# Priberam/Enhance-CB-Whisper

Measured on AMD Instinct MI355X. Metric: utterances/sec (30 s clips) + keywords/sec matched, Whisper-large-v3 LEF 10k kw, higher is better.
Workload: dtype bf16

## Files before the change

### enhance-cb-whisper_amd/csrc/cbw_kernels.h

```cpp
#pragma once
#include <hip/hip_runtime.h>
#include <stdint.h>

#include <initializer_list>
#include <string>

typedef __bf16 bf16;

enum {
    CBW_EPI_RELU = 1,
    CBW_EPI_GELU = 2,
    CBW_EPI_RES_F32 = 4,
    CBW_EPI_OUT_F32 = 8,
    CBW_EPI_RES_AFTER_ACT = 16,
    CBW_EPI_SPLIT3 = 32,
    CBW_EPI_RES_SPLIT = 64
};

struct ConvArgs {
    const void* x;
    const void* w;
    const float* bias;
    const void* res;
    void* y;
    const void* zero;
    int N, H, W, Cin, Ho, Wo, Cout, KH, KW;
    int sh, sw, ph, pw;
    int M;
    int res_ld, y_ld;
    int flags;
    const void* x2;
    int Cin2, H2, W2, s2;
    int ksplit;
    float* partial;
    float* y32;
    int x_ld, xfold;
};

hipError_t cbw_conv_igemm(const ConvArgs& a, hipStream_t st);
extern thread_local const char* cbw_last_conv_kernel;
extern thread_local int cbw_cs_grid_cus;
inline std::string kernel_name(const char* base, std::initializer_list<int> targs) {
    std::string s = std::string(base) + "<";
    bool first = true;
    for (int t : targs) {
        s += (first ? "" : ", ") + std::to_string(t);
        first = false;
    }
    return s + ">";
}
int cbw_conv_splitk_factor(const ConvArgs& a);
hipError_t cbw_conv_igemm_splitk(const ConvArgs& a, int ksplit, float* partial, hipStream_t st);
struct GemvArgs {
    const bf16* x;
    int ldx;
    const bf16* w;
    const float* bias;
    const void* res;
    int res_ld;
    void* y;
    int ldy;
    int M, N, K, flags;
    const float* xf;
    const float* ln_g;
    const float* ln_b;
    float ln_eps;
    bf16* kv_k;
    bf16* kv_v;
    int64_t kv_ld;
    int kv_D;
    const int* kv_pos;
    int kv_pos_rows;
};
int cbw_gemv_waves(int K);
bool cbw_gemv_ln_ok(int M, int K);
hipError_t cbw_gemv(const GemvArgs& a, hipStream_t st);

struct F8ConvArgs {
    const uint8_t* x;
    const uint8_t* w;
    const float* alpha;
    const float* bias;
    const uint8_t* res;
    float res_scale;
    void* y;
    float y_inv_scale;
    int out_bf16;
    const void* zero;
    int N, H, W, Cin, Ho, Wo, Cout, KH, KW, sh, sw, ph, pw, M;
    int relu;
};
bool cbw_conv_fp8_supported(const F8ConvArgs& a);
bool cbw_conv_fp8_stream_supported(const F8ConvArgs& a);
hipError_t cbw_conv_fp8_stream(const F8ConvArgs& a, hipStream_t st);
hipError_t cbw_conv_fp8(const F8ConvArgs& a, hipStream_t st);
hipError_t cbw_quant_fp8(const uint16_t* x, uint8_t* y, int64_t n, float inv_scale, hipStream_t st);
int cbw_absmax_groups();
hipError_t cbw_absmax_f32(const float* x, int64_t n, float* part, hipStream_t st);
hipError_t cbw_mfma_fp8_probe(const uint8_t* A, const uint8_t* Bt, float* C, int mode, hipStream_t st);
hipError_t cbw_cvt_fp8_probe(const float* x, uint8_t* q, float* back, int n, hipStream_t st);

bool cbw_conv_ring_supported(const ConvArgs& a);
hipError_t cbw_conv_ring(const ConvArgs& a, hipStream_t st);
bool cbw_conv_stream_supported(const ConvArgs& a);
bool cbw_conv_stream_wanted(const ConvArgs& a);
hipError_t cbw_conv_stream(const ConvArgs& a, hipStream_t st);
bool cbw_conv_chain_enabled();
bool cbw_conv_chain_supported(const ConvArgs& a, int red_cout);
hipError_t cbw_conv_chain_pack(const uint16_t* wr, uint16_t* packed, hipStream_t st);
hipError_t cbw_conv_chain(const ConvArgs& a, const uint16_t* wr_packed, const float* br, void* t1, hipStream_t st);

hipError_t cbw_bottleneck_s1(const uint16_t* x, uint16_t* y, const uint16_t* wr, const float* br, const uint16_t* wm,
                             const float* bm, const uint16_t* we, const float* be, const void* zero, int N, int H,
                             int W, hipStream_t st);
hipError_t cbw_bottleneck_s1_q8(const uint16_t* x, uint8_t* y, const uint16_t* wr, const float* br, const uint16_t* wm,
                                const float* bm, const uint16_t* we, const float* be, float inv_scale, int N, int H,
                                int W, hipStream_t st);
hipError_t cbw_bottleneck_s1_first(const uint16_t* x, uint16_t* y, const uint16_t* wr, const float* br,
                                   const uint16_t* wm, const float* bm, const uint16_t* wcat, const float* bcat,
                                   const void* zero, int N, int H, int W, hipStream_t st);

hipError_t cbw_cast_permute_lbtd(const float* x, uint16_t* y, int B, int L, int T, int D, hipStream_t st);
hipError_t cbw_normalize_rows(const void* x, int x_is_f32, void* y, int y_is_f32, int L, int B, int T, int E,
                              float eps, int permute_lb, hipStream_t st);
hipError_t cbw_nchw_to_nhwc4(const float* x, uint16_t* y, int K, int L, int H, int W, hipStream_t st);
hipError_t cbw_l2norm_rows_f32(float* x, int64_t rows, int E, hipStream_t st);
hipError_t cbw_lef_time_project(const float* x, const float* w, const float* b, void* y, int y_is_f32,
                                const float* mask_in, float* mask_out,
                                int L, int B, int T, int U, float eps, hipStream_t st);
hipError_t cbw_sim_maps(const uint16_t* kwd, const float* kwd_mask, const uint16_t* utt, const float* utt_mask,
                        uint16_t* out, int K, int L, int Tk, int Tu, int E, hipStream_t st);
hipError_t cbw_sim_maps_pairs(const uint16_t* kwd, const float* kwd_mask, int K, const uint16_t* utt,
                              const float* utt_mask, int B, const int32_t* pair_utt, const int32_t* pair_kwd, int p0,
                              uint16_t* out, int P, int L, int Tk, int Tu, int E, hipStream_t st);
hipError_t cbw_sim_to_nchw(const uint16_t* maps, float* out, int K, int L, int Tk, int Tu, hipStream_t st);
hipError_t cbw_stem_conv(const uint16_t* x, const uint16_t* w, const float* bias, uint16_t* y,
                         int N, int H, int W, int Ho, int Wo, hipStream_t st);
hipError_t cbw_stem_pool(const uint16_t* x, const uint16_t* w, const float* bias, uint16_t* y, int N, int H, int W,
                         int Hs, int Ws, int Hp, int Wp, hipStream_t st);
hipError_t cbw_stem16_pool(const uint16_t* x, const uint16_t* w, const float* bias, uint16_t* y, int N, int H,
                           int W, int Hs, int Ws, int Hp, int Wp, hipStream_t st);
hipError_t cbw_stem16_pool_x3(const uint16_t* x, const uint16_t* w, const float* bias, uint16_t* y, int N, int H,
                              int W, int Hs, int Ws, int Hp, int Wp, hipStream_t st);
hipError_t cbw_maps_split16(const float* x, uint16_t* y, int K, int L, int H, int W, hipStream_t st);
hipError_t cbw_sim_resize(const float* sim, int64_t layer_stride, int ld, const int* off_dev, int k0, int K, int L,
                          int Tu, int Ho, int Wo, uint16_t* out, hipStream_t st);
hipError_t cbw_nchw_to_nhwc16(const float* x, uint16_t* y, int K, int L, int H, int W, hipStream_t st);
hipError_t cbw_maxpool3s2(const uint16_t* x, uint16_t* y, int N, int H, int W, int C, int Ho, int Wo, hipStream_t st);
hipError_t cbw_pool_fc(const uint16_t* x, const float* w, const float* b, float* logits, int N, int HW, int C,
                       hipStream_t st);
int cbw_checksum_scratch_bytes();
hipError_t cbw_checksum64(const void* data, int64_t bytes, uint64_t* out, uint64_t* scratch, hipStream_t st);
hipError_t cbw_spot(const float* logits, const float* ghost, int K, float thr, float band, int mode, float* prob_out,
                    int* idx_out, int* n_out, hipStream_t st);

struct F32ConvArgs {
    const float* x;
    const float* w;
    const float* bias;
    const float* res;
    float* y;
    int N, H, W, Cin, Ho, Wo, Cout, KH, KW, sh, sw, ph, pw, M, relu;
};
hipError_t cbw_conv_f32(const F32ConvArgs& a, hipStream_t st);
hipError_t cbw_sim_f32(const float* kwd, const float* kwd_mask, const float* utt, const float* utt_mask, const int* sel,
                       int p0, int P, float* out, int L, int Tk, int Tu, int E, hipStream_t st);
hipError_t cbw_sim_f32_pairs(const float* kwd, const float* kwd_mask, int K, const float* utt, const float* utt_mask,
                             int B, const int32_t* pair_utt, const int32_t* pair_kwd, int n_pairs, const int* sel, int p0,
                             int P, float* out, int L, int Tk, int Tu, int E, hipStream_t st);
hipError_t cbw_sim_rows_f32(const float* utt, const float* kwd, const int* off, const int* sel, int p0, int P, int K,
                            int R, int L, int Tu, int D, int TkMax, int ld, float* rows, hipStream_t st);
hipError_t cbw_sim_resize_f32(const float* rows, const int* off, const int* sel, int p0, int P, int K, int R, int L,
                              int Tu, int TkMax, int ld, int Ho, int Wo, float* out, hipStream_t st);
hipError_t cbw_maxpool_f32(const float* x, float* y, int N, int H, int W, int C, int Ho, int Wo, hipStream_t st);
hipError_t cbw_pool_fc_f32(const float* x, const float* w, const float* b, const int* sel, int p0, int P, float* logits,
                           int HW, int C, hipStream_t st);
hipError_t cbw_permute_lbtd_f32(const float* x, float* y, int B, int L, int T, int D, hipStream_t st);
hipError_t cbw_split3(const float* x, uint16_t* y, int64_t M, int C, hipStream_t st);
hipError_t cbw_channel_sum_f32(const float* x, int64_t M, int C, float* part, hipStream_t st);
int cbw_channel_sum_groups();

constexpr int CBW_MEL_LONG_PARTS = 256;
hipError_t cbw_mel_frames(const float* pcm, int n_samples, const float* filters, const float* twiddle,
                          float* logmel, int n_mel, hipStream_t st, int L_pad = 0, int frames = 0);
hipError_t cbw_mel_finish(float* logmel, int n_mel, float* scratch, uint16_t* packed, int cpad, hipStream_t st,
                          int frames = 0);
hipError_t cbw_layernorm(const float* x, const float* g, const float* b, uint16_t* y, float* y32, int rows, int D,
                         float eps, hipStream_t st);
hipError_t cbw_attention(const uint16_t* qkv, uint16_t* out, int B, int T, int H, int hd, hipStream_t st);
// ... 32 lines not shown
```

### enhance-cb-whisper_amd/csrc/conv_igemm.hip

```cpp
#include "cbw_common.h"
#include "cbw_kernels.h"

thread_local const char* cbw_last_conv_kernel = "";

namespace {

constexpr int BK = 64;
constexpr int EPI_LD = 68;
constexpr int EPI_BYTES = 4 * 64 * EPI_LD * 4;
template <int BM, int BN>
constexpr int lds_bytes() { return 2 * (BM + BN) * 128 > EPI_BYTES ? 2 * (BM + BN) * 128 : EPI_BYTES; }

CBW_DEV int swz(int r) { return (r >> 1) & 7; }

CBW_DEV void store_out8(const ConvArgs& a, int flags, int m, int col, const float (&v)[8]) {
    if (flags & CBW_EPI_SPLIT3) {
        bf16x8 hi, lo;
#pragma unroll
        for (int q = 0; q < 8; ++q) {
            hi[q] = f2bf(v[q]);
            lo[q] = f2bf(v[q] - bf2f(hi[q]));
        }
        bf16* yp = (bf16*)a.y + (int64_t)m * a.y_ld + col;
        *(bf16x8*)yp = hi;
        *(bf16x8*)(yp + a.Cout) = lo;
        if (a.y32) {
            float* fp = a.y32 + (int64_t)m * a.Cout + col;
            *(f32x4*)fp = f32x4{v[0], v[1], v[2], v[3]};
            *(f32x4*)(fp + 4) = f32x4{v[4], v[5], v[6], v[7]};
        }
    } else if (flags & CBW_EPI_OUT_F32) {
        float* yp = (float*)a.y + (int64_t)m * a.y_ld + col;
        *(f32x4*)yp = f32x4{v[0], v[1], v[2], v[3]};
        *(f32x4*)(yp + 4) = f32x4{v[4], v[5], v[6], v[7]};
    } else {
        bf16x8 o;
#pragma unroll
        for (int q = 0; q < 8; ++q) o[q] = f2bf(v[q]);
        *(bf16x8*)((bf16*)a.y + (int64_t)m * a.y_ld + col) = o;
    }
}

CBW_DEV void res_split8(const ConvArgs& a, int m, int col, float (&rv)[8]) {
    const bf16* rp = (const bf16*)a.res + (int64_t)m * a.res_ld + col;
    const bf16x8 hi = *(const bf16x8*)rp, lo = *(const bf16x8*)(rp + a.Cout);
#pragma unroll
    for (int q = 0; q < 8; ++q) rv[q] = bf2f(hi[q]) + bf2f(lo[q]);
}

CBW_DEV int fold_c(int c0, int xfold) { return (xfold && c0 >= xfold) ? c0 - xfold : c0; }

template <int BM, int BN, int KH, int KW>
__global__ __launch_bounds__(256, 2) void conv_igemm_kernel(ConvArgs a) {
    static_assert((BM / 64) * (BN / 64) == 4, "4 waves x 64x64 tiles");
    static_assert(KH * KW <= 32, "tap mask");
    constexpr int STAGE = (BM + BN) * 128;
    constexpr int WN = BN / 64;
    constexpr int AR = BM / 32;
    constexpr int BR = BN / 32;
    extern __shared__ __attribute__((aligned(16))) char smem[];

    const int tid = threadIdx.x, lane = tid & 63, wid = tid >> 6;
    const int wm = wid / WN, wn = wid % WN;
    const int nt_n = a.Cout / BN;
    const int nt_m = (a.M + BM - 1) / BM;
    const int bid = xcd_remap(blockIdx.x, nt_m * nt_n);
    const int tm = bid / nt_n, tn = bid % nt_n;
    const int m0 = tm * BM, n0 = tn * BN;
    const int Ktot = KH * KW * a.Cin;
    const int csteps = a.Cin / BK;
    const int nsteps_all = KH * KW * csteps;
    const int HoWo = a.Ho * a.Wo;
    const int xld = a.x_ld ? a.x_ld : a.Cin;
    const int S = a.ksplit > 1 ? a.ksplit : 1;
    const int s_lo = (int)blockIdx.y * nsteps_all / S, s_hi = ((int)blockIdx.y + 1) * nsteps_all / S;

    const int sub_r = lane >> 3, chunk = lane & 7;
    const bf16* a_px[AR];
    unsigned a_tm[AR];
#pragma unroll
    for (int j = 0; j < AR; ++j) {
        const int r = (wid * AR + j) * 8 + sub_r;
        const int m = m0 + r;
        const bool okm = m < a.M;
        const int mm = okm ? m : 0;
        const int n = mm / HoWo, rem = mm - n * HoWo;
        const int oh = rem / a.Wo, ow = rem - oh * a.Wo;
        const int ih0 = oh * a.sh - a.ph, iw0 = ow * a.sw - a.pw;
        unsigned tm = 0;
#pragma unroll
        for (int kh = 0; kh < KH; ++kh)
#pragma unroll
            for (int kw = 0; kw < KW; ++kw) {
                const int ih = ih0 + kh, iw = iw0 + kw;
                if (okm && ih >= 0 && ih < a.H && iw >= 0 && iw < a.W) tm |= 1u << (kh * KW + kw);
            }
        a_tm[j] = tm;
        a_px[j] = (const bf16*)a.x + (int64_t)n * a.H * a.W * xld + ((int64_t)ih0 * a.W + iw0) * xld +
                  ((chunk ^ swz(r)) * 8);
    }
    int nx_cs = s_lo % csteps, nx_tap = s_lo / csteps;
    int nx_kh = nx_tap / KW, nx_kw = nx_tap - nx_kh * KW;
    const bf16* wrow[BR];
#pragma unroll
    for (int j = 0; j < BR; ++j) {
        const int r = (wid * BR + j) * 8 + sub_r;
        wrow[j] = (const bf16*)a.w + (int64_t)(n0 + r) * Ktot + ((chunk ^ swz(r)) * 8);
    }

    auto issue_stage = [&](int s, int buf) {
        const int tap = nx_tap;
        const int off = (nx_kh * a.W + nx_kw) * xld + fold_c(nx_cs * BK, a.xfold);
        if (++nx_cs == csteps) {
            nx_cs = 0;
            ++nx_tap;
            if (++nx_kw == KW) { nx_kw = 0; ++nx_kh; }
        }
        char* A = smem + buf * STAGE;
        char* B = A + BM * 128;
#pragma unroll
        for (int j = 0; j < AR; ++j) {
            const int rb = wid * AR + j;
            const void* src = ((a_tm[j] >> tap) & 1u) ? (const void*)(a_px[j] + off) : a.zero;
            __builtin_amdgcn_global_load_lds(src, (void*)(A + rb * 1024), 16, 0, 0);
        }
#pragma unroll
        for (int j = 0; j < BR; ++j) {
            const int rb = wid * BR + j;
            __builtin_amdgcn_global_load_lds((const void*)(wrow[j] + (int64_t)s * BK), (void*)(B + rb * 1024), 16, 0, 0);
        }
    };

    f32x4 acc[4][4];
#pragma unroll
    for (int i = 0; i < 4; ++i)
#pragma unroll
        for (int j = 0; j < 4; ++j) acc[i][j] = f32x4{0.f, 0.f, 0.f, 0.f};

    issue_stage(s_lo, 0);
    const int ecg = lane & 7, erow = lane >> 3;
    const int ecol = n0 + wn * 64 + ecg * 8;
    const bool res_bf16 = S == 1 && a.res != nullptr && !(a.flags & (CBW_EPI_RES_F32 | CBW_EPI_RES_SPLIT));
    bf16x8 rpre[8];
#pragma unroll
    for (int it = 0; it < 8; ++it) {
        const int m = m0 + wm * 64 + it * 8 + erow;
        if (res_bf16 && m < a.M)
            rpre[it] = *(const bf16x8*)((const bf16*)a.res + (int64_t)m * a.res_ld + ecol);
        else
            rpre[it] = bf16x8{};
    }
    f32x4 bias0 = {0.f, 0.f, 0.f, 0.f}, bias1 = {0.f, 0.f, 0.f, 0.f};
    if (a.bias) {
        bias0 = *(const f32x4*)(a.bias + ecol);
// ... 408 lines not shown
        for (int j = 0; j < BG; ++j)
            __builtin_amdgcn_global_load_lds((const void*)(wrow[j] + (int64_t)is_s * BIG_BK),
                                             (void*)(B + (j * 128 + wid * 16) * 64), 16, 0, 0);
        ++is_s;
        is_c += BIG_BK;
        if (is_c == a.Cin) {
            is_c = 0;
            ++is_tap;
            if (++is_kw == KW) { is_kw = 0; ++is_kh; }
        }
    };

    f32x4 acc[FM][4];
#pragma unroll
    for (int i = 0; i < FM; ++i)
#pragma unroll
        for (int j = 0; j < 4; ++j) acc[i][j] = f32x4{0.f, 0.f, 0.f, 0.f};

    issue_next();
    if (nsteps > 1) issue_next();
    if (nsteps > 2) issue_next();
    const int fr = lane & 15, fq = lane >> 4;
    for (int s = 0; s < nsteps; ++s) {
        if (s + 2 < nsteps) {
            if constexpr (G == 4) asm volatile("s_waitcnt vmcnt(8)" ::: "memory");
            else asm volatile("s_waitcnt vmcnt(6)" ::: "memory");
        } else if (s + 1 < nsteps) {
            if constexpr (G == 4) asm volatile("s_waitcnt vmcnt(4)" ::: "memory");
            else asm volatile("s_waitcnt vmcnt(3)" ::: "memory");
        } else {
            asm volatile("s_waitcnt vmcnt(0)" ::: "memory");
        }
        __builtin_amdgcn_s_barrier();
        const char* A = smem + (s & (BIG_NS - 1)) * STAGE;
        const char* B = A + BIG_BM * 64;
        bf16x8 av[FM], bv[4];
#pragma unroll
        for (int j = 0; j < 4; ++j) {
            const int r = wn * 64 + j * 16 + fr;
            bv[j] = *(const bf16x8*)(B + r * 64 + ((fq ^ swz4(r)) * 16));
        }
#pragma unroll
        for (int i = 0; i < FH; ++i) {
            const int r = wm * (FM * 16) + i * 16 + fr;
            av[i] = *(const bf16x8*)(A + r * 64 + ((fq ^ swz4(r)) * 16));
        }
#pragma unroll
        for (int i = 0; i < FH; ++i) {
            __builtin_amdgcn_sched_barrier(0);
            __builtin_amdgcn_s_setprio(1);
#pragma unroll
            for (int j = 0; j < 4; ++j)
                acc[i][j] = __builtin_amdgcn_mfma_f32_16x16x32_bf16(bv[j], av[i], acc[i][j], 0, 0, 0);
            __builtin_amdgcn_s_setprio(0);
            __builtin_amdgcn_sched_barrier(0);
            const int r = wm * (FM * 16) + (i + FH) * 16 + fr;
            av[i + FH] = *(const bf16x8*)(A + r * 64 + ((fq ^ swz4(r)) * 16));
        }
        __builtin_amdgcn_sched_barrier(0);
        if (s + 3 < nsteps) issue_next();
        __builtin_amdgcn_sched_barrier(0);
        __builtin_amdgcn_s_setprio(1);
#pragma unroll
        for (int i = FH; i < FM; ++i)
#pragma unroll
            for (int j = 0; j < 4; ++j)
                acc[i][j] = __builtin_amdgcn_mfma_f32_16x16x32_bf16(bv[j], av[i], acc[i][j], 0, 0, 0);
        __builtin_amdgcn_s_setprio(0);
        asm volatile("" ::: "memory");
    }

    const bool relu = a.flags & CBW_EPI_RELU;
    const bool split3 = a.flags & CBW_EPI_SPLIT3;
#pragma unroll
    for (int j = 0; j < 4; ++j) {
        const int col = n0 + wn * 64 + j * 16 + fq * 4;
        const f32x4 bb = a.bias ? *(const f32x4*)(a.bias + col) : f32x4{0.f, 0.f, 0.f, 0.f};
#pragma unroll
        for (int i = 0; i < FM; ++i) {
            const int m = m0 + wm * (FM * 16) + i * 16 + fr;
            if (m >= a.M) continue;
            f32x4 v;
#pragma unroll
            for (int q = 0; q < 4; ++q) {
                v[q] = acc[i][j][q] + bb[q];
                if (relu) v[q] = fmaxf(v[q], 0.f);
            }
            bf16x4 o;
#pragma unroll
            for (int q = 0; q < 4; ++q) o[q] = f2bf(v[q]);
            bf16* yp = (bf16*)a.y + (int64_t)m * a.y_ld + col;
            *(bf16x4*)yp = o;
            if (split3) {
                bf16x4 lo;
#pragma unroll
                for (int q = 0; q < 4; ++q) lo[q] = f2bf(v[q] - bf2f(o[q]));
                *(bf16x4*)(yp + a.Cout) = lo;
                if (a.y32) *(f32x4*)(a.y32 + (int64_t)m * a.Cout + col) = v;
            }
        }
    }
}

template <int BN, int KH, int KW>
hipError_t launch_big(const ConvArgs& a, hipStream_t st) {
    const int nt = ((a.M + BIG_BM - 1) / BIG_BM) * (a.Cout / BN);
    constexpr int lds = BIG_NS * (BIG_BM + BN) * 64;
    static const std::string nm = kernel_name("conv_igemm_big2", {BN, KH, KW});
    cbw_last_conv_kernel = nm.c_str();
    hipLaunchKernelGGL((conv_igemm_big2<BN, KH, KW>), dim3(nt), dim3(512), lds, st, a);
    return hipGetLastError();
}

constexpr int P8_BM = 256, P8_BN = 256, P8_BK = 64;
CBW_DEV int p8_off(int r, int c) { return r * 128 + ((c ^ ((r >> 1) & 7)) << 4); }
template <int BN> struct P8Shape {
    static constexpr int BM = 65536 / BN;
    static constexpr int NA = BM / 128, NB = BN / 128;
    static constexpr int WCN = BN / 64;
    static constexpr int BUF = (BM + BN) * 128;
};
template <int N> CBW_DEV void vm_wait() {
    static_assert(N >= 0 && N <= 15, "vm_wait");
    asm volatile("s_waitcnt vmcnt(%0)" ::"n"(N) : "memory");
}

template <int KH, int KW, int BN = 256>
__global__ __launch_bounds__(512, 1) void conv_igemm_p8(ConvArgs a) {
    static_assert(KH * KW <= 32, "tap mask");
    using S = P8Shape<BN>;
    constexpr int BM = S::BM, NA = S::NA, NB = S::NB, WCN = S::WCN;
    extern __shared__ __attribute__((aligned(16))) char smem[];
    const int tid = threadIdx.x, lane = tid & 63, wid = tid >> 6;
    const int wr = (wid >> 2) * (4 / WCN) + (wid & 3) / WCN, wc = (wid & 3) % WCN;
    const int fr = lane & 15, fq = lane >> 4;
    const int nt_n = a.Cout / BN;
    const int nt_m = (a.M + BM - 1) / BM;
    const int bid = xcd_remap(blockIdx.x, nt_m * nt_n);
    const int tm = bid / nt_n, tn = bid % nt_n;
    const int m0 = tm * BM, n0 = tn * BN;
    const int cin2 = a.x2 ? a.Cin2 : 0;
    const int Ktot = KH * KW * a.Cin + cin2;
    const int csteps = a.Cin / P8_BK;
    const int nk1 = KH * KW * csteps;
    const int nk = nk1 + cin2 / P8_BK;
    const int HoWo = a.Ho * a.Wo;
    const int xld = a.x_ld ? a.x_ld : a.Cin;

    const int sub = lane >> 3, pch = lane & 7;
    const bf16* a_px[2][NA];
    const bf16* a2_px[2][NA];
    unsigned a_tm[2][NA];
    const bf16* wrow[2][NB];
#pragma unroll
    for (int h = 0; h < 2; ++h)
#pragma unroll
        for (int g = 0; g < NA; ++g) {
            const int r = g * 128 + h * 64 + wid * 8 + sub;
            const int m = m0 + r;
            const bool okm = m < a.M;
            const int mm = okm ? m : 0;
            const int n = mm / HoWo, rem = mm - n * HoWo;
            const int oh = rem / a.Wo, ow = rem - oh * a.Wo;
            const int ih0 = oh * a.sh - a.ph, iw0 = ow * a.sw - a.pw;
            a2_px[h][g] = a.x2 ? (const bf16*)a.x2 + (((int64_t)n * a.H2 + oh * a.s2) * a.W2 + ow * a.s2) * cin2 +
                                     ((pch ^ ((r >> 1) & 7)) * 8)
                               : nullptr;
            unsigned tmask = 0;
#pragma unroll
            for (int kh = 0; kh < KH; ++kh)
#pragma unroll
                for (int kw = 0; kw < KW; ++kw) {
                    const int ih = ih0 + kh, iw = iw0 + kw;
                    if (okm && ih >= 0 && ih < a.H && iw >= 0 && iw < a.W) tmask |= 1u << (kh * KW + kw);
                }
            a_tm[h][g] = tmask;
            a_px[h][g] = (const bf16*)a.x + (int64_t)n * a.H * a.W * xld + ((int64_t)ih0 * a.W + iw0) * xld +
                         ((pch ^ ((r >> 1) & 7)) * 8);
        }
#pragma unroll
    for (int h = 0; h < 2; ++h)
#pragma unroll
        for (int g = 0; g < NB; ++g) {
            const int rb = h * (BN / 2) + g * 64 + wid * 8 + sub;
            const int rs = (rb & ~31) | (((rb & 15) >> 2) << 3) | (((rb >> 4) & 1) << 2) | (rb & 3);
            wrow[h][g] = (const bf16*)a.w + (int64_t)(n0 + rs) * Ktot + ((pch ^ ((rb >> 1) & 7)) * 8);
        }
    int nx_cs = 0, nx_tap = 0, nx_kh = 0, nx_kw = 0;
    int nx_off = fold_c(0, a.xfold);
    auto advance = [&]() {
        if (++nx_cs == csteps) {
            nx_cs = 0;
            ++nx_tap;
            if (++nx_kw == KW) { nx_kw = 0; ++nx_kh; }
        }
        nx_off = (nx_kh * a.W + nx_kw) * xld + fold_c(nx_cs * P8_BK, a.xfold);
    };
    auto issue = [&](int kt, int which) {
        char* A = smem + (kt & 1) * S::BUF;
        if (which == 0 || which == 3) {
            const int h = which == 3;
            if (kt >= nk1) {
                const int c0 = (kt - nk1) * P8_BK;
#pragma unroll
                for (int g = 0; g < NA; ++g) {
                    const void* src = (a_tm[h][g] & 1u) ? (const void*)(a2_px[h][g] + c0) : a.zero;
                    __builtin_amdgcn_global_load_lds(src, (void*)(A + (g * 128 + h * 64 + wid * 8) * 128), 16, 0, 0);
                }
                return;
            }
            const int tap = nx_tap;
            const int toff = nx_off;
#pragma unroll
            for (int g = 0; g < NA; ++g) {
                const void* src = ((a_tm[h][g] >> tap) & 1u) ? (const void*)(a_px[h][g] + toff) : a.zero;
                __builtin_amdgcn_global_load_lds(src, (void*)(A + (g * 128 + h * 64 + wid * 8) * 128), 16, 0, 0);
            }
        } else {
            const int h = which - 1;
            char* B = A + BM * 128;
#pragma unroll
            for (int g = 0; g < NB; ++g)
                __builtin_amdgcn_global_load_lds((const void*)(wrow[h][g] + (int64_t)kt * P8_BK),
                                                 (void*)(B + (h * (BN / 2) + g * 64 + wid * 8) * 128), 16, 0, 0);
        }
    };

    f32x4 acc[8][4];
#pragma unroll
    for (int i = 0; i < 8; ++i)
#pragma unroll
        for (int j = 0; j < 4; ++j) acc[i][j] = f32x4{0.f, 0.f, 0.f, 0.f};
    bf16x8 av[4][2], bv[2][2];

#pragma unroll
    for (int w = 0; w < 4; ++w) issue(0, w);
    advance();
    asm volatile("s_waitcnt vmcnt(0)" ::: "memory");
    __builtin_amdgcn_s_barrier();
    if (wid >= 4) __builtin_amdgcn_s_barrier();
    for (int kt = 0; kt < nk; ++kt) {
        const char* A = smem + (kt & 1) * S::BUF;
        const char* B = A + BM * 128;
        const bool more = kt + 1 < nk;
#pragma unroll
        for (int q = 0; q < 4; ++q) {
            const int mi = q >> 1, ni = (q == 1 || q == 2) ? 1 : 0;
            __builtin_amdgcn_sched_barrier(0);
            if (more) {
                issue(kt + 1, q);
                if (q == 3) advance();
                if (q == 0) vm_wait<2 * NA>();
                else if (q == 2) vm_wait<2 * NB>();
                else vm_wait<NA + NB>();
            } else if (q == 0) {
                vm_wait<NA>();
            } else {
                vm_wait<0>();
            }
            if (q == 0 || q == 2) {
#pragma unroll
                for (int i = 0; i < 4; ++i)
#pragma unroll
                    for (int ks = 0; ks < 2; ++ks)
                        av[i][ks] = *(const bf16x8*)(A + p8_off(wr * 128 + mi * 64 + i * 16 + fr, ks * 4 + fq));
            }
            if (q != 2) {
#pragma unroll
                for (int j = 0; j < 2; ++j)
#pragma unroll
                    for (int ks = 0; ks < 2; ++ks)
                        bv[j][ks] = *(const bf16x8*)(B + p8_off(ni * (BN / 2) + wc * 32 + j * 16 + fr, ks * 4 + fq));
            }
            __builtin_amdgcn_sched_barrier(0);
            __builtin_amdgcn_s_barrier();
            __builtin_amdgcn_s_setprio(1);
#pragma unroll
            for (int ks = 0; ks < 2; ++ks)
#pragma unroll
                for (int i = 0; i < 4; ++i)
#pragma unroll
                    for (int j = 0; j < 2; ++j)
                        acc[mi * 4 + i][ni * 2 + j] =
                            __builtin_amdgcn_mfma_f32_16x16x32_bf16(bv[j][ks], av[i][ks], acc[mi * 4 + i][ni * 2 + j], 0, 0, 0);
            __builtin_amdgcn_s_setprio(0);
            __builtin_amdgcn_sched_barrier(0);
            __builtin_amdgcn_s_barrier();
        }
    }
    if (wid < 4) __builtin_amdgcn_s_barrier();

    const int flags = a.flags;
    const bool relu = flags & CBW_EPI_RELU;
    const bool has_res = a.res != nullptr;
    const bool res_split = flags & CBW_EPI_RES_SPLIT, res_f32 = flags & CBW_EPI_RES_F32;
#pragma unroll
    for (int ni = 0; ni < 2; ++ni) {
        const int col = n0 + ni * (BN / 2) + wc * 32 + fq * 8;
        f32x4 bb[2] = {f32x4{0.f, 0.f, 0.f, 0.f}, f32x4{0.f, 0.f, 0.f, 0.f}};
        if (a.bias) {
            bb[0] = *(const f32x4*)(a.bias + col);
            bb[1] = *(const f32x4*)(a.bias + col + 4);
        }
        uint4 rw0[8], rw1[8];
        if (has_res) {
#pragma unroll
            for (int f = 0; f < 8; ++f) {
                const int mc = min(m0 + wr * 128 + f * 16 + fr, a.M - 1);
                if (res_f32) {
                    const float* rp = (const float*)a.res + (int64_t)mc * a.res_ld + col;
                    rw0[f] = *(const uint4*)rp;
                    rw1[f] = *(const uint4*)(rp + 4);
                } else {
                    const bf16* rp = (const bf16*)a.res + (int64_t)mc * a.res_ld + col;
                    rw0[f] = *(const uint4*)rp;
                    if (res_split) rw1[f] = *(const uint4*)(rp + a.Cout);
                }
            }
        }
#pragma unroll
        for (int f = 0; f < 8; ++f) {
            const int m = m0 + wr * 128 + f * 16 + fr;
            if (m >= a.M) continue;
            float v[8];
#pragma unroll
            for (int j = 0; j < 2; ++j)
#pragma unroll
                for (int q = 0; q < 4; ++q) v[4 * j + q] = acc[f][ni * 2 + j][q] + bb[j][q];
            if (has_res) {
                float rv[8];
                if (res_split) {
                    const bf16x8 hi = __builtin_bit_cast(bf16x8, rw0[f]), lo = __builtin_bit_cast(bf16x8, rw1[f]);
#pragma unroll
                    for (int q = 0; q < 8; ++q) rv[q] = bf2f(hi[q]) + bf2f(lo[q]);
                } else if (res_f32) {
                    const f32x4 r0 = __builtin_bit_cast(f32x4, rw0[f]), r1 = __builtin_bit_cast(f32x4, rw1[f]);
#pragma unroll
                    for (int q = 0; q < 4; ++q) { rv[q] = r0[q]; rv[q + 4] = r1[q]; }
                } else {
                    const bf16x8 r = __builtin_bit_cast(bf16x8, rw0[f]);
#pragma unroll
                    for (int q = 0; q < 8; ++q) rv[q] = bf2f(r[q]);
                }
#pragma unroll
                for (int q = 0; q < 8; ++q) v[q] += rv[q];
            }
            if (relu)
#pragma unroll
                for (int q = 0; q < 8; ++q) v[q] = fmaxf(v[q], 0.f);
            store_out8(a, flags, m, col, v);
        }
    }
}

template <int KH, int KW, int BN = 256>
hipError_t launch_p8(const ConvArgs& a, hipStream_t st) {
    using S = P8Shape<BN>;
    if (BN != 256) {
        static const hipError_t attr = hipFuncSetAttribute((const void*)conv_igemm_p8<KH, KW, BN>,
                                                           hipFuncAttributeMaxDynamicSharedMemorySize, 2 * S::BUF);
        if (attr != hipSuccess) return attr;
    }
    static const std::string nm = kernel_name("conv_igemm_p8", {KH, KW, BN});
    cbw_last_conv_kernel = nm.c_str();
    const int nt = ((a.M + S::BM - 1) / S::BM) * (a.Cout / BN);
    hipLaunchKernelGGL((conv_igemm_p8<KH, KW, BN>), dim3(nt), dim3(512), 2 * S::BUF, st, a);
    return hipGetLastError();
}

int p8_x2() {
    const char* e = getenv("CBW_P8_X2");
    return e ? atoi(e) : 1;
}

bool p8_tier_enabled() {
    const char* e = getenv("CBW_P8_TIER");
    return !(e && atoi(e) == 0);
}

int p8_n128() {
    const char* e = getenv("CBW_P8_N128");
    return e ? atoi(e) : 1;
}

int p8_mode() {
    const char* e = getenv("CBW_CONV_P8");
    return e ? atoi(e) : 1;
}

int num_cus() {
    static int n = 0;
    if (n == 0) {
        int dev = 0;
        (void)hipGetDevice(&dev);
        if (hipDeviceGetAttribute(&n, hipDeviceAttributeMultiprocessorCount, dev) != hipSuccess || n <= 0) n = 256;
    }
    return n;
}

template <int BM, int BN, int KH, int KW>
hipError_t launch_persist(const ConvArgs& a, hipStream_t st) {
    const int ntiles = ((a.M + BM - 1) / BM) * (a.Cout / BN);
    int G = 2 * num_cus();
    if (ntiles < G) G = ntiles;
    constexpr int lds = 2 * (BM + BN) * 128 + 4 * 8 * EPI_LD * 4;
    static const std::string nm = kernel_name("conv_igemm_persist", {BM, BN, KH, KW});
    cbw_last_conv_kernel = nm.c_str();
    hipLaunchKernelGGL((conv_igemm_persist<BM, BN, KH, KW>), dim3(G), dim3(256), lds, st, a, ntiles);
    return hipGetLastError();
}

template <int BM, int BN, int KH, int KW>
hipError_t launch_t(const ConvArgs& a, hipStream_t st) {
    const int nt = ((a.M + BM - 1) / BM) * (a.Cout / BN);
    constexpr int lds = lds_bytes<BM, BN>();
    static const std::string nm = kernel_name("conv_igemm_kernel", {BM, BN, KH, KW});
    cbw_last_conv_kernel = nm.c_str();
    hipLaunchKernelGGL((conv_igemm_kernel<BM, BN, KH, KW>), dim3(nt), dim3(256), lds, st, a);
    return hipGetLastError();
}

bool ring_wanted(const ConvArgs& a) {
    if (!cbw_conv_ring_supported(a)) return false;
    const int ktot = a.KH * a.KW * a.Cin + (a.x2 ? a.Cin2 : 0);
    return a.KH * a.KW == 1 && a.res == nullptr && ktot <= 768;
}

template <int KH, int KW>
hipError_t launch_k(const ConvArgs& a, hipStream_t st) {
    const int64_t xld = a.x_ld ? a.x_ld : a.Cin;
    if (((int64_t)(KH - 1) * a.W + (KW - 1)) * xld + a.Cin + (a.x2 ? a.Cin2 : 0) > INT32_MAX) return hipErrorInvalidValue;
    const bool tile_only = a.xfold || (a.x_ld && a.x_ld != a.Cin) || (a.flags & (CBW_EPI_SPLIT3 | CBW_EPI_RES_SPLIT));
    const bool p8_fit = p8_mode() == 1 && a.res == nullptr && a.Cout % P8_BN == 0 && a.Cin % P8_BK == 0 &&
                        a.xfold % P8_BK == 0 && KH * KW * a.Cin + (a.x2 ? a.Cin2 : 0) >= 512 &&
                        (a.x2 == nullptr || (KH * KW == 1 && a.Cin2 % P8_BK == 0 && !a.xfold && !a.x_ld)) &&
                        !(a.flags & (CBW_EPI_OUT_F32 | CBW_EPI_GELU | CBW_EPI_RES_SPLIT)) &&
                        ((a.M + P8_BM - 1) / P8_BM) * (a.Cout / P8_BN) >= num_cus();
    const int px2 = p8_x2();
    if (p8_fit && a.x2 && px2 >= 2) return launch_p8<KH, KW>(a, st);
    if (!tile_only && KH * KW == 1 && cbw_conv_stream_wanted(a)) return cbw_conv_stream(a, st);
    if (p8_fit && a.x2 && px2 >= 1) return launch_p8<KH, KW>(a, st);
    if (p8_tier_enabled() && (a.flags & (CBW_EPI_SPLIT3 | CBW_EPI_OUT_F32)) && a.xfold && a.x2 == nullptr &&
        p8_mode() == 1 && a.Cout % P8_BN == 0 && a.Cin % P8_BK == 0 && a.xfold % P8_BK == 0 &&
        !(a.flags & (CBW_EPI_GELU | CBW_EPI_RES_AFTER_ACT))) {
        const int ktot = KH * KW * a.Cin;
        const int tiles = ((a.M + P8_BM - 1) / P8_BM) * (a.Cout / P8_BN);
        if (ktot >= 512 && (tiles >= num_cus() || (ktot >= 4096 && 2 * tiles >= num_cus())))
            return launch_p8<KH, KW>(a, st);
    }
    if (!tile_only && ring_wanted(a)) return cbw_conv_ring(a, st);
    const bool big_ok = a.res == nullptr && a.x2 == nullptr &&
                        !(a.flags & (CBW_EPI_OUT_F32 | CBW_EPI_GELU | CBW_EPI_RES_SPLIT)) &&
                        a.Cin % BIG_BK == 0 && a.xfold % BIG_BK == 0 && KH * KW * a.Cin >= 256;
    const int big_tiles = ((a.M + BIG_BM - 1) / BIG_BM) * (a.Cout / 256);
    if (big_ok && big_tiles >= num_cus()) {
        if (a.Cout % 256 == 0 && p8_mode() == 1 && a.Cin % P8_BK == 0 && a.xfold % P8_BK == 0)
            return launch_p8<KH, KW>(a, st);
        if (a.Cout % 256 == 0) return launch_big<256, KH, KW>(a, st);
    }
    if (big_ok && p8_n128() && p8_mode() == 1 && a.Cout % 256 == 128 && a.Cin % P8_BK == 0 && a.xfold % P8_BK == 0 &&
        KH * KW * a.Cin >= 512 && ((a.M + 511) / 512) * (a.Cout / 128) >= num_cus())
        return launch_p8<KH, KW, 128>(a, st);
    if (a.Cout % 128 == 0) {
        const bool short_k = a.KH * a.KW * (a.Cin / BK) == 1;
        if (a.x2 != nullptr || short_k || a.res != nullptr)
            return launch_persist<128, 128, KH, KW>(a, st);
        return launch_t<128, 128, KH, KW>(a, st);
    }
    if (a.x2 != nullptr) return hipErrorInvalidValue;
    return launch_t<256, 64, KH, KW>(a, st);
}

}

namespace {
__global__ __launch_bounds__(256) void splitk_epilogue_kernel(ConvArgs a, int S) {
    const int64_t n4 = (int64_t)a.M * a.Cout / 4;
    for (int64_t e = blockIdx.x * (int64_t)blockDim.x + threadIdx.x; e < n4; e += (int64_t)gridDim.x * blockDim.x) {
        const int64_t i = e * 4;
        const int m = (int)(i / a.Cout), col = (int)(i - (int64_t)m * a.Cout);
        f32x4 v = *(const f32x4*)(a.partial + i);
        for (int z = 1; z < S; ++z) v += *(const f32x4*)(a.partial + (int64_t)z * a.M * a.Cout + i);
        if (a.bias) v += *(const f32x4*)(a.bias + col);
        float rv[4] = {0.f, 0.f, 0.f, 0.f};
        const bool has_res = a.res != nullptr;
        if (has_res) {
            if (a.flags & CBW_EPI_RES_F32) {
                const f32x4 r = *(const f32x4*)((const float*)a.res + (int64_t)m * a.res_ld + col);
#pragma unroll
                for (int q = 0; q < 4; ++q) rv[q] = r[q];
            } else {
                const bf16x4 r = *(const bf16x4*)((const bf16*)a.res + (int64_t)m * a.res_ld + col);
#pragma unroll
                for (int q = 0; q < 4; ++q) rv[q] = bf2f(r[q]);
            }
            if (!(a.flags & CBW_EPI_RES_AFTER_ACT))
#pragma unroll
                for (int q = 0; q < 4; ++q) v[q] += rv[q];
        }
#pragma unroll
        for (int q = 0; q < 4; ++q) {
            if (a.flags & CBW_EPI_RELU) v[q] = fmaxf(v[q], 0.f);
            else if (a.flags & CBW_EPI_GELU) v[q] = gelu_erf(v[q]);
            if (has_res && (a.flags & CBW_EPI_RES_AFTER_ACT)) v[q] += rv[q];
        }
        if (a.flags & CBW_EPI_OUT_F32) {
            *(f32x4*)((float*)a.y + (int64_t)m * a.y_ld + col) = v;
        } else {
            bf16x4 o;
#pragma unroll
// ... 43 lines not shown
```

Baseline: 6.107.

## Remap p8 conv tile rows by output-row groups to skip padded kernel rows

Reorders the implicit-GEMM M dimension in the p8 conv kernel so each tile holds output pixels from the same output row(s) across a group of images. A per-row pixel table is kept in LDS. Each tile then computes which kernel rows (kh) touch only zero padding and restricts its K loop to the valid kh range, skipping MFMA work on boundary rows. The epilogue maps the permuted rows back to their original output indices for the residual load and the store. This adds LDS setup, extra syncs and scattered output writes, and only helps tiles that sit on the top or bottom image border.

```diff
diff --git a/enhance-cb-whisper_amd/csrc/cbw_kernels.h b/enhance-cb-whisper_amd/csrc/cbw_kernels.h
--- a/enhance-cb-whisper_amd/csrc/cbw_kernels.h
+++ b/enhance-cb-whisper_amd/csrc/cbw_kernels.h
@@ -35,6 +35,7 @@
     float* partial;
     float* y32;
     int x_ld, xfold;
+    int p8_g;
 };
 
 hipError_t cbw_conv_igemm(const ConvArgs& a, hipStream_t st);
diff --git a/enhance-cb-whisper_amd/csrc/conv_igemm.hip b/enhance-cb-whisper_amd/csrc/conv_igemm.hip
--- a/enhance-cb-whisper_amd/csrc/conv_igemm.hip
+++ b/enhance-cb-whisper_amd/csrc/conv_igemm.hip
@@ -1,5 +1,6 @@
 #include "cbw_common.h"
 #include "cbw_kernels.h"
+#include "p8_rowmap.h"
 
 thread_local const char* cbw_last_conv_kernel = "";
 
@@ -714,16 +715,49 @@
     const bf16* a2_px[2][NA];
     unsigned a_tm[2][NA];
     const bf16* wrow[2][NB];
+    constexpr bool ROWS = KH * KW > 1;
+    bool rowmap = false;
+    int kh_lo = 0, kt_lo = 0, kt_hi = nk;
+    if constexpr (ROWS) {
+        rowmap = a.p8_g > 0;
+        if (rowmap) {
+            if (tid < BM) {
+                int4 rec{-1, 0, 0, 0};
+                if (m0 + tid < a.M) p8_row_pixel(m0 + tid, a.N, a.Ho, a.Wo, a.p8_g, rec.x, rec.y, rec.z, rec.w);
+                ((int4*)smem)[tid] = rec;
+            }
+            __syncthreads();
+            const int4 first = ((const int4*)smem)[0], last = ((const int4*)smem)[min(BM, a.M - m0) - 1];
+            int kh_hi;
+            p8_kh_range(__builtin_amdgcn_readfirstlane(first.y), __builtin_amdgcn_readfirstlane(last.y),
+                        __builtin_amdgcn_readfirstlane(first.w) == __builtin_amdgcn_readfirstlane(last.w), a.H, a.sh,
+                        a.ph, KH, kh_lo, kh_hi);
+            kt_lo = kh_lo * KW * csteps;
+            kt_hi = kh_hi * KW * csteps;
+        }
+    }
 #pragma unroll
     for (int h = 0; h < 2; ++h)
 #pragma unroll
         for (int g = 0; g < NA; ++g) {
             const int r = g * 128 + h * 64 + wid * 8 + sub;
-            const int m = m0 + r;
-            const bool okm = m < a.M;
-            const int mm = okm ? m : 0;
-            const int n = mm / HoWo, rem = mm - n * HoWo;
-            const int oh = rem / a.Wo, ow = rem - oh * a.Wo;
+            bool okm;
+            int n, oh, ow;
+            if (ROWS && rowmap) {
+                const int4 rec = ((const int4*)smem)[r];
+                okm = rec.x >= 0;
+                n = okm ? rec.x : 0;
+                oh = rec.y;
+                ow = rec.z;
+            } else {
+                const int m = m0 + r;
+                okm = m < a.M;
+                const int mm = okm ? m : 0;
+                n = mm / HoWo;
+                const int rem = mm - n * HoWo;
+                oh = rem / a.Wo;
+                ow = rem - oh * a.Wo;
+            }
             const int ih0 = oh * a.sh - a.ph, iw0 = ow * a.sw - a.pw;
             a2_px[h][g] = a.x2 ? (const bf16*)a.x2 + (((int64_t)n * a.H2 + oh * a.s2) * a.W2 + ow * a.s2) * cin2 +
                                      ((pch ^ ((r >> 1) & 7)) * 8)
@@ -749,7 +783,12 @@
             wrow[h][g] = (const bf16*)a.w + (int64_t)(n0 + rs) * Ktot + ((pch ^ ((rb >> 1) & 7)) * 8);
         }
     int nx_cs = 0, nx_tap = 0, nx_kh = 0, nx_kw = 0;
-    int nx_off = fold_c(0, a.xfold);
+    if constexpr (ROWS) {
+        nx_kh = kh_lo;
+        nx_tap = nx_kh * KW;
+        if (rowmap) __syncthreads();
+    }
+    int nx_off = nx_kh * a.W * xld + fold_c(0, a.xfold);
     auto advance = [&]() {
         if (++nx_cs == csteps) {
             nx_cs = 0;
@@ -796,15 +835,15 @@
     bf16x8 av[4][2], bv[2][2];
 
 #pragma unroll
-    for (int w = 0; w < 4; ++w) issue(0, w);
+    for (int w = 0; w < 4; ++w) issue(kt_lo, w);
     advance();
     asm volatile("s_waitcnt vmcnt(0)" ::: "memory");
     __builtin_amdgcn_s_barrier();
     if (wid >= 4) __builtin_amdgcn_s_barrier();
-    for (int kt = 0; kt < nk; ++kt) {
+    for (int kt = kt_lo; kt < kt_hi; ++kt) {
         const char* A = smem + (kt & 1) * S::BUF;
         const char* B = A + BM * 128;
-        const bool more = kt + 1 < nk;
+        const bool more = kt + 1 < kt_hi;
 #pragma unroll
         for (int q = 0; q < 4; ++q) {
             const int mi = q >> 1, ni = (q == 1 || q == 2) ? 1 : 0;
@@ -856,6 +895,23 @@
     const bool relu = flags & CBW_EPI_RELU;
     const bool has_res = a.res != nullptr;
     const bool res_split = flags & CBW_EPI_RES_SPLIT, res_f32 = flags & CBW_EPI_RES_F32;
+    if constexpr (ROWS) {
+        if (rowmap) {
+            if (tid < BM) {
+                int n, oh, ow, grp, m = -1;
+                if (m0 + tid < a.M) {
+                    p8_row_pixel(m0 + tid, a.N, a.Ho, a.Wo, a.p8_g, n, oh, ow, grp);
+                    m = (n * a.Ho + oh) * a.Wo + ow;
+                }
+                ((int*)smem)[tid] = m;
+            }
+            __syncthreads();
+        }
+    }
+    auto row_m = [&](int f) {
+        if (ROWS && rowmap) return ((const int*)smem)[wr * 128 + f * 16 + fr];
+        return m0 + wr * 128 + f * 16 + fr;
+    };
 #pragma unroll
     for (int ni = 0; ni < 2; ++ni) {
         const int col = n0 + ni * (BN / 2) + wc * 32 + fq * 8;
@@ -868,7 +924,7 @@
         if (has_res) {
 #pragma unroll
             for (int f = 0; f < 8; ++f) {
-                const int mc = min(m0 + wr * 128 + f * 16 + fr, a.M - 1);
+                const int mc = (ROWS && rowmap) ? max(row_m(f), 0) : min(row_m(f), a.M - 1);
                 if (res_f32) {
                     const float* rp = (const float*)a.res + (int64_t)mc * a.res_ld + col;
                     rw0[f] = *(const uint4*)rp;
@@ -882,8 +938,8 @@
         }
 #pragma unroll
         for (int f = 0; f < 8; ++f) {
-            const int m = m0 + wr * 128 + f * 16 + fr;
-            if (m >= a.M) continue;
+            const int m = row_m(f);
+            if ((ROWS && rowmap) ? m < 0 : m >= a.M) continue;
             float v[8];
 #pragma unroll
             for (int j = 0; j < 2; ++j)
@@ -915,9 +971,20 @@
     }
 }
 
+int p8_rowgroup(const ConvArgs& a, int BM) {
+    const char* e = getenv("CBW_P8_ROWSKIP");
+    if ((e && atoi(e) == 0) || a.N <= 0 || (int64_t)a.N * a.Ho * a.Wo != a.M) return 0;
+    const char* ge = getenv("CBW_P8_ROWGROUP");
+    int G = ge ? atoi(ge) : 0;
+    if (G <= 0) G = p8_default_rowgroup(a.Wo, BM);
+    return G < a.N ? G : a.N;
+}
+
 template <int KH, int KW, int BN = 256>
-hipError_t launch_p8(const ConvArgs& a, hipStream_t st) {
+hipError_t launch_p8(const ConvArgs& a0, hipStream_t st) {
     using S = P8Shape<BN>;
+    ConvArgs a = a0;
+    a.p8_g = KH * KW > 1 ? p8_rowgroup(a, S::BM) : 0;
     if (BN != 256) {
         static const hipError_t attr = hipFuncSetAttribute((const void*)conv_igemm_p8<KH, KW, BN>,
                                                            hipFuncAttributeMaxDynamicSharedMemorySize, 2 * S::BUF);
diff --git a/enhance-cb-whisper_amd/csrc/p8_rowmap.h b/enhance-cb-whisper_amd/csrc/p8_rowmap.h
--- /dev/null
+++ b/enhance-cb-whisper_amd/csrc/p8_rowmap.h
@@ -0,0 +1,40 @@
+#pragma once
+
+#if defined(__HIPCC__)
+#define CBW_HD __host__ __device__ __forceinline__
+#else
+#define CBW_HD inline
+#endif
+
+CBW_HD void p8_row_pixel(int L, int N, int Ho, int Wo, int G, int& n, int& oh, int& ow, int& grp) {
+    if (G > N) G = N;
+    grp = L / (G * Ho * Wo);
+    const int l = L - grp * (G * Ho * Wo);
+    const int left = N - grp * G;
+    const int rowlen = (left < G ? left : G) * Wo;
+    oh = l / rowlen;
+    const int rem = l - oh * rowlen;
+    const int p = rem / Wo;
+    ow = rem - p * Wo;
+    n = grp * G + p;
+}
+
+CBW_HD void p8_kh_range(int oh_first, int oh_last, bool same_group, int H, int sh, int ph, int KH, int& kh_lo,
+                        int& kh_hi) {
+    kh_lo = 0;
+    kh_hi = KH;
+    if (!same_group) return;
+    const int lo = ph - oh_last * sh, hi = H + ph - oh_first * sh;
+    const int clo = lo > 0 ? lo : 0, chi = hi < KH ? hi : KH;
+    if (clo < chi) {
+        kh_lo = clo;
+        kh_hi = chi;
+    }
+}
+
+inline int p8_default_rowgroup(int Wo, int BM) {
+    for (int G = 1; G <= 64; ++G)
+        if ((G * Wo) % BM == 0) return G;
+    const int G = 9 * BM / Wo;
+    return G > 0 ? G : 1;
+}
```

New measurement: 6.187, median of 6. 1.01x the previous value.
